# Rayhane-mamah/Tacotron-2

Hardware: NVIDIA H100
Metric: wavenet_train_audio_samples_per_sec (higher is better)
Workload: dtype bf16

## Files before the change

### tacotron-2_b200/csrc/t2_gemm.cu

```cuda
#include <stdlib.h>
#include <mutex>

#include "t2_gemm.cuh"
#include "t2_gemm.h"

namespace t2 {

static long long* g_timing_buffer = nullptr;
void set_timing_buffer(long long* p) { g_timing_buffer = p; }

typedef CUresult (*EncodeTiledFn)(CUtensorMap*, CUtensorMapDataType, cuuint32_t, void*, const cuuint64_t*,
                                  const cuuint64_t*, const cuuint32_t*, const cuuint32_t*,
                                  CUtensorMapInterleave, CUtensorMapSwizzle, CUtensorMapL2promotion,
                                  CUtensorMapFloatOOBfill);

static EncodeTiledFn get_encode_fn() {
  static EncodeTiledFn fn = nullptr;
  static std::once_flag once;
  std::call_once(once, [] {
    void* p = nullptr;
    cudaDriverEntryPointQueryResult q;
    if (cudaGetDriverEntryPoint("cuTensorMapEncodeTiled", &p, cudaEnableDefault, &q) == cudaSuccess &&
        q == cudaDriverEntryPointSuccess)
      fn = reinterpret_cast<EncodeTiledFn>(p);
// ... 110 lines not shown
    T2_REQUIRE(mc > 0, T2_ERR_UNSUPPORTED_SHAPE, "act_gemm: clusters of %d CTAs cannot be scheduled on this device", cs);
  }
  T2_CHECK_CUDA(cudaLaunchKernelEx(&cfg, act_gemm_kernel<EPI, BN>, g));
  t2_count_launch();
  return T2_OK;
}

int make_gemm_args(int epi, int BN, const ActGemmCall& c, GemmArgs& g, dim3& grid, int& cs) {
  T2_REQUIRE(c.na >= 1 && c.na <= 4 && c.nseg >= 1 && c.nseg <= kMaxSeg, T2_ERR_INVALID_ARG,
             "act_gemm: bad map/segment count (%d, %d)", c.na, c.nseg);
  T2_REQUIRE(c.cluster == 0 || c.cluster == 1 || c.cluster == 2 || c.cluster == 4 || c.cluster == 8, T2_ERR_INVALID_ARG,
             "act_gemm: cluster size must be 0 (default), 1, 2, 4 or 8 (got %d)", c.cluster);
  int ktot = 0;
  for (int s = 0; s < c.nseg; ++s) {
    T2_REQUIRE(c.seg[s].map >= 0 && c.seg[s].map < c.na && c.seg[s].nkb > 0 && c.seg[s].nlayers > 0,
               T2_ERR_INVALID_ARG, "act_gemm: bad segment %d", s);
    ktot += c.seg[s].nkb * c.seg[s].nlayers * kBK;
  }
  T2_REQUIRE(c.w_k0 + ktot <= ((c.wK + kBK - 1) / kBK) * kBK, T2_ERR_INVALID_ARG,
             "act_gemm: segments cover K=%d but packed weight has K=%d", ktot, c.wK);
  if (c.ksplit > 1) {
    T2_REQUIRE(epi == EPI_TOUT && c.ksplit * kBK <= ktot, T2_ERR_INVALID_ARG,
               "act_gemm: split-K needs an atomically accumulating epilogue and at least one k-block per slice");
    const bool use0 = c.epi.ptr[0] && c.epi.i[0] > 0, use1 = c.epi.ptr[1] && c.epi.i[3] > c.epi.i[0];
    T2_REQUIRE((!use0 || c.epi.i[2] == 2) && (!use1 || c.epi.i[5] == 2), T2_ERR_INVALID_ARG,
               "act_gemm: split-K needs atomic accumulation (mode 2) into every destination in use (modes %d, %d)", c.epi.i[2],
               c.epi.i[5]);
  }
  memset(&g, 0, sizeof(g));
  for (int i = 0; i < 4; ++i) {
    int rc = encode_act_map(&g.amap[i], c.a[i < c.na ? i : 0], kBM);
    if (rc) return rc;
  }
  grid = dim3((c.T + kBM - 1) / kBM * c.B, c.n_tiles, c.ksplit > 1 ? c.ksplit : 1);
  cs = pick_cluster(BN, grid, c.cluster);
  int rc = encode_wt_map(&g.bmap, c.w, c.wN, c.wK, c.wL, BN / cs);
  if (rc) return rc;
  for (int s = 0; s < c.nseg; ++s) g.seg[s] = c.seg[s];
  g.nseg = c.nseg;
  g.T = c.T;
  g.tiles_per_b = (c.T + kBM - 1) / kBM;
  g.b_layer = c.w_layer;
  g.b_k0 = c.w_k0;
  g.dbg = g_timing_buffer;
  g.epi = c.epi;
  if (!c.epi.i[11]) {
    const void* outs[3] = {nullptr, nullptr, nullptr};
    int ldo = 0;
    if (epi == EPI_GATE) { outs[0] = c.epi.ptr[0]; outs[1] = c.epi.ptr[1]; outs[2] = c.epi.ptr[2]; ldo = c.epi.i[0]; }
    else if (epi == EPI_RES) { outs[0] = c.epi.ptr[1]; outs[1] = c.epi.ptr[2]; ldo = BN; }
    else if (epi == EPI_GATE_BWD) { outs[0] = c.epi.ptr[2]; ldo = 2 * c.epi.i[0]; }
    else if (epi == EPI_DX) { outs[0] = c.epi.ptr[1]; ldo = BN; }
    for (int i = 0; i < 3; ++i)
      if (outs[i]) {
        rc = encode_out_map(&g.omap[i], outs[i], ldo, c.T, c.B);
        if (rc) return rc;
      }
  }
  return T2_OK;
}

long long* take_timing_slice(long long n_slots) {
  long long* p = g_timing_buffer;
  if (p) g_timing_buffer = p + n_slots;
  return p;
}

int launch_act_gemm(int epi, int BN, const ActGemmCall& c, cudaStream_t stream, int* cluster_used) {
  GemmArgs g;
  dim3 grid;
  int cs = 1;
  const int rc = make_gemm_args(epi, BN, c, g, grid, cs);
  if (rc) return rc;
  if (cluster_used) *cluster_used = cs;
#define T2_CASE(E, N) \
  if (epi == E && BN == N) return launch_one<E, N>(g, grid, cs, stream);
  T2_CASE(EPI_GATE, 256)
  T2_CASE(EPI_RES, 128)
  T2_CASE(EPI_RES, 256)
  T2_CASE(EPI_BIAS_ACT, 128)
  T2_CASE(EPI_BIAS_ACT, 256)
  T2_CASE(EPI_CE, 256)
  T2_CASE(EPI_SCALE_RELUMASK, 128)
  T2_CASE(EPI_SCALE_RELUMASK, 256)
  T2_CASE(EPI_GATE_BWD, 128)
  T2_CASE(EPI_GATE_BWD, 256)
  T2_CASE(EPI_DX, 128)
  T2_CASE(EPI_DX, 256)
  T2_CASE(EPI_MOL, 32)
  T2_CASE(EPI_LSTM, 32)
  T2_CASE(EPI_TOUT, 32)
#undef T2_CASE
  return t2_set_error(T2_ERR_UNSUPPORTED_SHAPE, "act_gemm: no kernel for epilogue %d with BN=%d", epi, BN);
}

int launch_wgrad(const ActT* maps, int nmaps, const WgradTile* tiles_dev, int ntiles, float* out, int T,
                 int B, cudaStream_t stream) {
  T2_REQUIRE(nmaps >= 1 && nmaps <= 6 && ntiles >= 1, T2_ERR_INVALID_ARG, "wgrad: bad map/tile count");
  WgradArgs g;
  memset(&g, 0, sizeof(g));
  for (int i = 0; i < 6; ++i) {
    int rc = encode_act_map(&g.map[i], maps[i < nmaps ? i : 0], kBK);
    if (rc) return rc;
  }
  g.tiles = tiles_dev;
  g.out = out;
  g.T = T;
  g.B = B;
  static bool configured = false;
  if (!configured) {
    T2_CHECK_CUDA(cudaFuncSetAttribute(wgrad_gemm_kernel, cudaFuncAttributeMaxDynamicSharedMemorySize, kWgSmemBytes));
    configured = true;
  }
  cudaLaunchConfig_t cfg;
  memset(&cfg, 0, sizeof(cfg));
  cfg.gridDim = dim3(ntiles); cfg.blockDim = dim3(kGemmThreads); cfg.dynamicSmemBytes = kWgSmemBytes; cfg.stream = stream;
  cudaLaunchAttribute attr[1];
  attr[0].id = cudaLaunchAttributeProgrammaticStreamSerialization;
  attr[0].val.programmaticStreamSerializationAllowed = 1;
  cfg.attrs = attr; cfg.numAttrs = pdl_enabled() ? 1 : 0;
  T2_CHECK_CUDA(cudaLaunchKernelEx(&cfg, wgrad_gemm_kernel, g));
  t2_count_launch();
  return T2_OK;
}

void append_wgrad_tiles(std::vector<WgradTile>& v, const WgradTile& proto, int a_ch0, int Ca, int b_ch0, int Cb, long long out_off,
                        int ldc) {
  for (int m0 = 0; m0 < Ca; m0 += kWgBM)
    for (int n0 = 0; n0 < Cb; n0 += kWgBN) {
      WgradTile t;
      memset(&t, 0, sizeof(t));
      t.a_map = proto.a_map; t.a_ch0 = a_ch0 + m0; t.a_shift = proto.a_shift; t.a_layer = proto.a_layer;
      t.b_map = proto.b_map; t.b_ch0 = b_ch0 + n0; t.b_shift = proto.b_shift; t.b_layer = proto.b_layer;
      t.out_off = out_off + (long long)m0 * ldc + n0; t.ldc = ldc;
      t.m_valid = Ca - m0 < kWgBM ? Ca - m0 : kWgBM;
      t.n_valid = Cb - n0 < kWgBN ? Cb - n0 : kWgBN;
      t.scale = proto.scale; t.accumulate = proto.accumulate; t.div = proto.div;
      v.push_back(t);
    }
}

constexpr long long kChainTimeoutNs = 1000000000LL;

__device__ __forceinline__ int ld_acquire_gpu(const int* p) {
  int v;
  asm volatile("ld.acquire.gpu.global.b32 %0, [%1];" : "=r"(v) : "l"(p) : "memory");
  return v;
}
__device__ __forceinline__ void red_release_gpu_add(int* p, int v) {
  asm volatile("red.release.gpu.global.add.s32 [%0], %1;" ::"l"(p), "r"(v) : "memory");
}
__device__ __forceinline__ void fence_proxy_async_global() { asm volatile("fence.proxy.async.global;" ::: "memory"); }

template <int BN>
__device__ __forceinline__ void chain_init_barriers(uint8_t* smem) {
  using Cfg = ActGemmCfg<BN>;
  uint64_t* full_bar = reinterpret_cast<uint64_t*>(smem + Cfg::kPipeBytes + Cfg::kEpiBytes);
  for (int i = 0; i < Cfg::kStages; ++i) {
    mbar_init(&full_bar[i], 1);
    mbar_init(&full_bar[Cfg::kStages + i], kActEpiWarps);
  }
  fence_barrier_init();
}
template <int BN>
__device__ __forceinline__ void chain_inval_barriers(uint8_t* smem) {
  using Cfg = ActGemmCfg<BN>;
  uint64_t* full_bar = reinterpret_cast<uint64_t*>(smem + Cfg::kPipeBytes + Cfg::kEpiBytes);
  for (int i = 0; i < 2 * Cfg::kStages; ++i)
    asm volatile("mbarrier.inval.shared::cta.b64 [%0];" ::"r"(smem_u32(&full_bar[i])) : "memory");
}

template <bool FWD, int BN0, int BN1>
__global__ void __launch_bounds__(kActGemmThreads, 1) wn_chain_kernel(const __grid_constant__ ChainArgs a) {
  constexpr int E0 = FWD ? EPI_GATE : EPI_GATE_BWD, E1 = FWD ? EPI_RES : EPI_DX;
  using C0 = ActGemmCfg<BN0>;
  using C1 = ActGemmCfg<BN1>;
  static_assert(C0::kPipeBytes == C1::kPipeBytes && C0::kEpiBytes == C1::kEpiBytes && C0::kSmemBytes == C1::kSmemBytes,
                "both GEMMs of a chain share one shared-memory plan");
  extern __shared__ uint8_t smem_raw[];
  uint8_t* smem = reinterpret_cast<uint8_t*>((reinterpret_cast<uintptr_t>(smem_raw) + 1023) & ~uintptr_t(1023));
  __shared__ EpiArgs s_epi;
  __shared__ int s_ticket;
  int* done = a.ctr + 16;
  int* stop = a.ctr + 1;
  int prev_kind = -1;
  for (;;) {
    if (threadIdx.x == 0) {
      int t = atomicAdd(a.ctr, 1);
      if (t < a.n_tix && *reinterpret_cast<volatile int*>(stop) == 0) {
        long long* dbg = a.dbg ? a.dbg + size_t(t) * kDbgSlots : nullptr;
        const long long t_start = globaltimer_ns();
        if (dbg) { dbg[0] = t_start; dbg[3] = smid(); }
        const ChainTicket k = a.tix[t];
        for (int i = k.dep_lo; i <= k.dep_hi && t < a.n_tix; ++i)
          while (ld_acquire_gpu(done + i) < k.dep_target) {
            if (globaltimer_ns() - t_start > kChainTimeoutNs) {
              if (atomicExch(stop, 1) == 0) atomicAdd(a.err, 1);
              t = a.n_tix;
              break;
            }
            __nanosleep(32);
          }
        fence_proxy_async_global();
        if (dbg) dbg[1] = globaltimer_ns();
        EpiArgs e = a.args[k.kind * a.L + k.layer].epi;
        if (FWD && k.kind == 0 && !a.save) { e.ptr[0] = nullptr; e.ptr[1] = nullptr; }
        if (FWD && k.kind == 1) e.ptr[3] = const_cast<float*>(a.params) + reinterpret_cast<uintptr_t>(e.ptr[3]);
        if (k.kind == 1) { e.seed = a.seed; e.ptr[7] = const_cast<unsigned long long*>(a.d_step); }
        s_epi = e;
        if (prev_kind == 0) chain_inval_barriers<BN0>(smem);
        else if (prev_kind == 1) chain_inval_barriers<BN1>(smem);
        if (k.kind == 0) chain_init_barriers<BN0>(smem);
        else chain_init_barriers<BN1>(smem);
        prev_kind = k.kind;
      } else {
        t = a.n_tix;
      }
      s_ticket = t;
    }
    __syncthreads();
    const int t = s_ticket;
    if (t >= a.n_tix) break;
    const ChainTicket k = a.tix[t];
    const GemmArgs& g = a.args[k.kind * a.L + k.layer];
    int all_kb = 0;
    for (int s = 0; s < g.nseg; ++s) all_kb += g.seg[s].nkb * g.seg[s].nlayers;
    if ((threadIdx.x >> 5) == kActEpiWarps) {
      fence_proxy_async_global();
      asm volatile("fence.proxy.async.shared::cta;" ::: "memory");
    }
    if (k.kind == 0) act_gemm_tile<E0, BN0, true>(g, s_epi, smem, k.m, k.n, 0, all_kb, 1, 0, 1, nullptr);
    else act_gemm_tile<E1, BN1, true>(g, s_epi, smem, k.m, k.n, 0, all_kb, 1, 0, 1, nullptr);
    fence_proxy_async_global();
    __syncthreads();
    if (threadIdx.x == 0) {
      red_release_gpu_add(done + k.done, 1);
      if (a.dbg) a.dbg[size_t(t) * kDbgSlots + 2] = globaltimer_ns();
    }
  }
}

template <bool FWD, int BN0, int BN1>
int launch_chain_kernel(const ChainArgs& a, int grid, cudaStream_t st) {
  static bool configured = false;
  if (!configured) {
    T2_CHECK_CUDA(cudaFuncSetAttribute(wn_chain_kernel<FWD, BN0, BN1>, cudaFuncAttributeMaxDynamicSharedMemorySize,
                                       ActGemmCfg<BN0>::kSmemBytes));
    configured = true;
  }
  wn_chain_kernel<FWD, BN0, BN1><<<grid, kActGemmThreads, ActGemmCfg<BN0>::kSmemBytes, st>>>(a);
  t2_count_launch();
  T2_CHECK_CUDA(cudaGetLastError());
  return T2_OK;
}


int launch_wn_chain(bool fwd, int bn0, int bn1, const ChainArgs& a, int grid, cudaStream_t st) {
  if (fwd && bn0 == 256) return bn1 == 256 ? launch_chain_kernel<true, 256, 256>(a, grid, st) : launch_chain_kernel<true, 256, 128>(a, grid, st);
  if (!fwd && bn0 == 256) return bn1 == 256 ? launch_chain_kernel<false, 256, 256>(a, grid, st) : launch_chain_kernel<false, 256, 128>(a, grid, st);
  if (!fwd && bn0 == 128) return bn1 == 256 ? launch_chain_kernel<false, 128, 256>(a, grid, st) : launch_chain_kernel<false, 128, 128>(a, grid, st);
  return t2_set_error(T2_ERR_UNSUPPORTED_SHAPE, "layer chain: no kernel for %s with BN %d / %d", fwd ? "forward" : "backward", bn0, bn1);
}

}
```

### tacotron-2_b200/csrc/t2_gemm.cuh

```cuda
#pragma once
#include "t2_common.cuh"
#include "t2_gemm_types.h"

namespace t2 {

__device__ __forceinline__ void store_bf16x32(__nv_bfloat16* dst, const float (&v)[32]) {
  uint4* d = reinterpret_cast<uint4*>(dst);
#pragma unroll
  for (int q = 0; q < 4; ++q) {
    uint4 u;
    u.x = pack_bf16x2(v[q * 8 + 0], v[q * 8 + 1]);
    u.y = pack_bf16x2(v[q * 8 + 2], v[q * 8 + 3]);
    u.z = pack_bf16x2(v[q * 8 + 4], v[q * 8 + 5]);
    u.w = pack_bf16x2(v[q * 8 + 6], v[q * 8 + 7]);
    d[q] = u;
  }
}
__device__ __forceinline__ void load_bf16x32(const __nv_bfloat16* src, float (&v)[32]) {
  const uint4* s = reinterpret_cast<const uint4*>(src);
#pragma unroll
  for (int q = 0; q < 4; ++q) {
    uint4 u = __ldg(s + q);
    v[q * 8 + 0] = bf16lo(u.x); v[q * 8 + 1] = bf16hi(u.x);
    v[q * 8 + 2] = bf16lo(u.y); v[q * 8 + 3] = bf16hi(u.y);
// ... 718 lines not shown
  static __device__ __forceinline__ void run(const EpiArgs& e, const EpiCtx& c) {
    const int R = BN;
    const __nv_bfloat16* dxo = static_cast<const __nv_bfloat16*>(e.ptr[0]);
    const float rs = e.f[0], p = e.f[1];
    const float keep_inv = 1.f / (1.f - p);
    const unsigned long long seed = e.seed + (e.ptr[7] ? *static_cast<const unsigned long long*>(e.ptr[7]) : 0ull);
    const uint32_t hs = hash_seed(seed, uint32_t(e.i[1]));
    const size_t row = (size_t(c.b) * c.T + c.t) * R;
    if (BN == 256 && dxo) tile_fill_sw<kCoherent>(c.tile(1), dxo + c.row0 * BN + 128, BN, c.nrows, c);
#pragma unroll 1
    for (int gq = 0; gq < BN / 128; ++gq) {
      uint8_t* tile = c.tile(gq == 0 ? 2 : 1);
      const int cq = c.cg;
      const int j0 = gq * 128 + cq * 32;
      float acc[32], g[32];
      acc_ld32f(c.trow + j0, acc);
      if (p > 0.f) {
        const uint32_t thr = uint32_t(p * 65536.f);
#pragma unroll
        for (int j = 0; j < 32; j += 2) {
          const uint32_t h = hash_bits32(hs, (row + j0 + j) >> 1);
          acc[j] = (h & 0xFFFFu) >= thr ? acc[j] * keep_inv : 0.f;
          acc[j + 1] = (h >> 16) >= thr ? acc[j + 1] * keep_inv : 0.f;
        }
      }
      if (dxo) {
        stage_get_sw(tile, c.lane, cq, g);
#pragma unroll
        for (int j = 0; j < 32; ++j) acc[j] += rs * g[j];
      }
      stage_put_sw(tile, c.lane, cq, acc);
      tile_store(tile, c.omap + 0, gq * 128, c);
      if (e.ptr[2]) {
        const float cs = warp_colsum32(acc, c.lane);
        fx_add(static_cast<long long*>(e.ptr[2]) + j0 + colsum32_col(c.lane), cs * e.f[2]);
      }
    }
  }
};

template <>
struct Epilogue<EPI_LSTM, 32> {
  static __device__ __forceinline__ void run(const EpiArgs& e, const EpiCtx& c) {
    const int H = e.i[0], nb = e.i[1];
    float* ex = reinterpret_cast<float*>(c.smem_all);
    const int q = c.qbar - 1;
    if (c.cg == 0) {
      float v[32];
      acc_ld32f(c.trow, v);
#pragma unroll
      for (int j = 0; j < 32; ++j) ex[(q * 32 + c.lane) * 33 + j] = v[j];
    }
    asm volatile("bar.sync 5, 512;\n" ::: "memory");
    const float* pre = static_cast<const float*>(e.ptr[0]);
    const float* bias = static_cast<const float*>(e.ptr[1]);
    const float* c_prev = static_cast<const float*>(e.ptr[2]);
    float* c_out = static_cast<float*>(e.ptr[3]);
    const __nv_bfloat16* h_prev = static_cast<const __nv_bfloat16*>(e.ptr[4]);
    __nv_bfloat16* h_state = static_cast<__nv_bfloat16*>(e.ptr[5]);
    __nv_bfloat16* h_out = static_cast<__nv_bfloat16*>(e.ptr[6]);
    __nv_bfloat16* gst = static_cast<__nv_bfloat16*>(e.ptr[7]);
    __nv_bfloat16* tst = static_cast<__nv_bfloat16*>(e.ptr[8]);
    const int* lens = static_cast<const int*>(e.ptr[9]);
    const unsigned long long seed = e.seed + (e.ptr[10] ? *static_cast<const unsigned long long*>(e.ptr[10]) : 0ull);
    const uint32_t hs_c = hash_seed(seed, uint32_t(e.i[8]) * 2u), hs_h = hash_seed(seed, uint32_t(e.i[8]) * 2u + 1u);
    const float z = e.f[0];
    const int t = e.i[7];
    const int etid = (c.cg * 4 + q) * 32 + c.lane;
    const int u0 = c.m_tile * 32, b0 = c.n_tile * 32;
#pragma unroll 1
    for (int p = etid; p < 1024; p += 512) {
      const int bl = p >> 5, ul = p & 31;
      const int b = b0 + bl, u = u0 + ul;
      if (b >= nb || u >= H) continue;
      float zi = ex[(0 * 32 + ul) * 33 + bl], zj = ex[(1 * 32 + ul) * 33 + bl];
      float zf = ex[(2 * 32 + ul) * 33 + bl], zo = ex[(3 * 32 + ul) * 33 + bl];
      if (pre) {
        const float* pr = pre + size_t(b) * e.i[3];
        zi += pr[u]; zj += pr[H + u]; zf += pr[2 * H + u]; zo += pr[3 * H + u];
      }
      if (bias) { zi += bias[u]; zj += bias[H + u]; zf += bias[2 * H + u]; zo += bias[3 * H + u]; }
      float gi = sigmoidf_(zi), gj = tanhf_(zj), gf = sigmoidf_(zf + 1.f), go = sigmoidf_(zo);
      const float cp = c_prev[size_t(b) * H + u];
      const float hp = __bfloat162float(h_prev[size_t(b) * e.i[4] + u]);
      const float cn = gf * cp + gi * gj;
      const float tc = tanhf_(cn);
      const float hn = go * tc;
      const bool live = lens ? (t < lens[b]) : true;
      float cs, hsv, ho = hn;
      if (e.i[9]) {
        const uint64_t idx = (uint64_t(t) * nb + b) * H + u;
        cs = (z <= 0.f || hash_uniform32(hs_c, idx) >= z) ? cn : cp;
        hsv = (z <= 0.f || hash_uniform32(hs_h, idx) >= z) ? hn : hp;
      } else {
        cs = (1.f - z) * cn + z * cp;
        hsv = (1.f - z) * hn + z * hp;
      }
      float tcs = tc;
      if (!live) { cs = cp; hsv = hp; ho = 0.f; gi = gj = gf = go = 0.f; tcs = 0.f; }
      c_out[size_t(b) * H + u] = cs;
      h_state[size_t(b) * e.i[5] + u] = __float2bfloat16(hsv);
      h_out[size_t(b) * e.i[6] + u] = __float2bfloat16(ho);
      if (gst) {
        __nv_bfloat16* g = gst + size_t(b) * 4 * H;
        g[u] = __float2bfloat16(gi); g[H + u] = __float2bfloat16(gj);
        g[2 * H + u] = __float2bfloat16(gf); g[3 * H + u] = __float2bfloat16(go);
      }
      if (tst) tst[size_t(b) * H + u] = __float2bfloat16(tcs);
    }
  }
};

template <>
struct Epilogue<EPI_TOUT, 32> {
  static __device__ __forceinline__ void run(const EpiArgs& e, const EpiCtx& c) {
    if (c.cg != 0) return;
    const int k = c.t, nb = e.i[6];
    float v[32];
    acc_ld32f(c.trow, v);
    float* dst; int ld, acc, kk;
    if (k < e.i[0]) { dst = static_cast<float*>(e.ptr[0]); ld = e.i[1]; acc = e.i[2]; kk = k; }
    else if (k < e.i[3]) { dst = static_cast<float*>(e.ptr[1]); ld = e.i[4]; acc = e.i[5]; kk = k - e.i[0]; }
    else return;
    if (!dst) return;
#pragma unroll
    for (int j = 0; j < 32; ++j) {
      const int b = c.n_tile * 32 + j;
      if (b < nb) {
        float* d = dst + size_t(b) * ld + kk;
        if (acc == 2) atomicAdd(d, v[j]);
        else *d = acc ? *d + v[j] : v[j];
      }
    }
  }
};

template <int BN>
struct ActGemmCfg {
  static constexpr int kABytes = kBM * kBK * 2;
  static constexpr int kBBytes = BN * kBK * 2;
  static constexpr int kStageBytes = kABytes + kBBytes;
  static constexpr int kAccBytes = kBM * BN * 4;
  static constexpr int kEpiBytes = 4 * kSTileBytes;
  static constexpr int kTailBytes = 8 * kSTileBytes;
  static constexpr int kPipeBudget = 232448 - kEpiBytes - 1024  - 256 ;
  static constexpr int kStages = kPipeBudget / kStageBytes > 6 ? 6 : kPipeBudget / kStageBytes;
  static constexpr int kPipeBytes =
      kStages * kStageBytes > kAccBytes + kTailBytes ? kStages * kStageBytes : kAccBytes + kTailBytes;
  static constexpr int kSmemBytes = kPipeBytes + kEpiBytes + 1024 + 256;
  static_assert(kStages >= 2 && kPipeBytes <= kPipeBudget && kSmemBytes <= 232448, "shared memory budget");
  static_assert(kPipeBytes % 1024 == 0, "staging tiles must be aligned to the 1024-byte swizzle atom");
};

template <int EPI, int BN, bool kChain = false>
__device__ __forceinline__ void act_gemm_tile(const GemmArgs& g, const EpiArgs& epi, uint8_t* smem, int m_tile, int n_tile,
                                              int kb_lo, int kb_hi, uint32_t cs, uint32_t crank, uint16_t cmask, long long* dbg) {
  using Cfg = ActGemmCfg<BN>;
  constexpr int WN = BN / 2;
  float* acc_s = reinterpret_cast<float*>(smem);
  uint8_t* staging = smem + Cfg::kPipeBytes - Cfg::kTailBytes;
  uint64_t* full_bar = reinterpret_cast<uint64_t*>(smem + Cfg::kPipeBytes + Cfg::kEpiBytes);
  uint64_t* empty_bar = full_bar + Cfg::kStages;
  const int warp = threadIdx.x >> 5;
  const int b = m_tile / g.tiles_per_b;
  const int t0 = (m_tile - b * g.tiles_per_b) * kBM;
  const int total_kb = kb_hi - kb_lo;

  if (warp == kActEpiWarps) {
    if (elect_one()) {
      int stage = 0;
      uint32_t phase = 0;
      int kb_global = 0;
      for (int s = 0; s < g.nseg; ++s) {
        const Seg sg = g.seg[s];
        for (int l = 0; l < sg.nlayers; ++l) {
          for (int kb = 0; kb < sg.nkb; ++kb, ++kb_global) {
            if (kb_global < kb_lo || kb_global >= kb_hi) continue;
            mbar_wait(&empty_bar[stage], phase ^ 1);
            mbar_expect_tx(&full_bar[stage], Cfg::kStageBytes);
            uint8_t* sa = smem + stage * Cfg::kStageBytes;
            uint8_t* sb = sa + Cfg::kABytes;
            tma_load_4d(sa, &g.amap[sg.map], &full_bar[stage], sg.k0 + kb * kBK, t0 + sg.shift, b, sg.layer0 + l);
            if (cs == 1) {
              tma_load_3d(sb, &g.bmap, &full_bar[stage], g.b_k0 + kb_global * kBK, n_tile * BN, g.b_layer);
            } else {
              const int rows = BN / int(cs);
              tma_load_3d_mc(sb + crank * rows * (kBK * 2), &g.bmap, &full_bar[stage], g.b_k0 + kb_global * kBK,
                             n_tile * BN + int(crank) * rows, g.b_layer, cmask);
            }
            if (++stage == Cfg::kStages) { stage = 0; phase ^= 1; }
          }
        }
      }
    }
  } else {
    const int q = warp & 3;
    const int lane = threadIdx.x & 31;
    EpiCtx c;
    c.lane = lane;
    c.cg = warp >> 2;
    c.qbar = 1 + q;
    c.b = b; c.T = g.T;
    const int tw = t0 + q * 32;
    c.t = tw + c.lane;
    c.valid = c.t < g.T;
    c.row0 = size_t(b) * g.T + tw;
    c.nrows = g.T - tw < 0 ? 0 : (g.T - tw > 32 ? 32 : g.T - tw);
    c.stg = staging + q * kSTileBytes;
    c.smem_all = smem + Cfg::kAccBytes;
    c.m_tile = m_tile;
    c.omap = g.omap; c.tq = tw; c.sk = 0;
    c.n_tile = n_tile;
    constexpr bool kCoh = EPI == EPI_RES || EPI == EPI_DX;
    if constexpr (kCoh) Epilogue<EPI, BN>::template prefetch<kChain>(epi, c);
    else if constexpr (EpiHasPrefetch<EPI>::value) Epilogue<EPI, BN>::prefetch(epi, c);

    const int wg = warp >> 2, mh = wg >> 1, nh = wg & 1;
    float d[WN / 2];
#pragma unroll
    for (int i = 0; i < WN / 2; ++i) d[i] = 0.f;
    int stage = 0, prev = 0;
    uint32_t phase = 0;
    for (int kb = 0; kb < total_kb; ++kb) {
      mbar_wait(&full_bar[stage], phase);
      __syncwarp();
      if (dbg && kb == 0 && threadIdx.x == 0) dbg[2] = clock64();
      const uint32_t sa = smem_u32(smem + stage * Cfg::kStageBytes) + uint32_t(mh * 64 * 128);
      const uint32_t sb = smem_u32(smem + stage * Cfg::kStageBytes + Cfg::kABytes) + uint32_t(nh * WN * 128);
      const uint64_t adesc = make_gdesc_sw128(sa, 16, 1024);
      const uint64_t bdesc = make_gdesc_sw128(sb, 16, 1024);
      wgmma_fence();
      wgmma_fence_regs(d);
#pragma unroll
      for (int k = 0; k < kBK / 16; ++k)
        Wgmma<WN, 0, 0>::mma(d, adesc + uint64_t(k * 2), bdesc + uint64_t(k * 2), (kb > 0 || k > 0) ? 1u : 0u);
      wgmma_commit();
      wgmma_fence_regs(d);
      wgmma_wait<1>();
      if (kb > 0 && lane == 0) {
        if (cs == 1) mbar_arrive(&empty_bar[prev]);
        else for (uint32_t r = 0; r < cs; ++r) mbar_arrive_cluster(&empty_bar[prev], r);
      }
      prev = stage;
      if (++stage == Cfg::kStages) { stage = 0; phase ^= 1; }
    }
    wgmma_wait<0>();
    wgmma_fence_regs(d);
    if (dbg && threadIdx.x == 0) dbg[3] = clock64();
    asm volatile("bar.sync 6, 512;\n" ::: "memory");
    {
      const int r0 = mh * 64 + (warp & 3) * 16 + (lane >> 2);
#pragma unroll
      for (int j = 0; j < WN / 8; ++j)
#pragma unroll
        for (int i = 0; i < 2; ++i) {
          const int r = r0 + 8 * i, col = nh * WN + 8 * j + 2 * (lane & 3);
          *reinterpret_cast<float2*>(acc_s + r * BN + ((((col >> 2) ^ (r & 7)) << 2) | (col & 3))) =
              make_float2(d[4 * j + 2 * i], d[4 * j + 2 * i + 1]);
        }
    }
    asm volatile("bar.sync 6, 512;\n" ::: "memory");
    const int row = q * 32 + lane;
    c.trow = AccRow{acc_s + row * BN, 0, row & 7};
    if (dbg && threadIdx.x == 0) dbg[4] = clock64();
    if constexpr (kCoh) Epilogue<EPI, BN>::template run<kChain>(epi, c);
    else Epilogue<EPI, BN>::run(epi, c);
    if (dbg && threadIdx.x == 0) dbg[5] = clock64();
    tile_store_drain(c);
  }
}

template <int EPI, int BN>
__global__ void __launch_bounds__(kActGemmThreads, 1) act_gemm_kernel(const __grid_constant__ GemmArgs g) {
  using Cfg = ActGemmCfg<BN>;
  constexpr int WN = BN / 2;
  extern __shared__ uint8_t smem_raw[];
  uint8_t* smem = reinterpret_cast<uint8_t*>((reinterpret_cast<uintptr_t>(smem_raw) + 1023) & ~uintptr_t(1023));
  float* acc_s = reinterpret_cast<float*>(smem);
  uint8_t* staging = smem + Cfg::kPipeBytes - Cfg::kTailBytes;
  uint64_t* full_bar = reinterpret_cast<uint64_t*>(smem + Cfg::kPipeBytes + Cfg::kEpiBytes);
  uint64_t* empty_bar = full_bar + Cfg::kStages;

  const int warp = threadIdx.x >> 5;
  const int m_tile = blockIdx.x;
  const uint32_t cs = cluster_nctarank(), crank = cluster_ctarank();
  const uint16_t cmask = uint16_t((1u << cs) - 1u);
  long long* dbg = g.dbg ? g.dbg + ((size_t(blockIdx.z) * gridDim.y + blockIdx.y) * gridDim.x + blockIdx.x) * kDbgSlots : nullptr;
  if (dbg && threadIdx.x == 0) { dbg[0] = clock64(); dbg[8] = globaltimer_ns(); dbg[11] = smid(); }
  const int b = m_tile / g.tiles_per_b;
  const int t0 = (m_tile - b * g.tiles_per_b) * kBM;

  int all_kb = 0;
  for (int s = 0; s < g.nseg; ++s) all_kb += g.seg[s].nkb * g.seg[s].nlayers;
  const int kb_lo = int((long long)all_kb * blockIdx.z / gridDim.z), kb_hi = int((long long)all_kb * (blockIdx.z + 1) / gridDim.z);
  const int total_kb = kb_hi - kb_lo;

  if (warp == kActEpiWarps && elect_one()) {
    for (int i = 0; i < 4; ++i) tma_prefetch_desc(&g.amap[i]);
    tma_prefetch_desc(&g.bmap);
    for (int i = 0; i < Cfg::kStages; ++i) {
      mbar_init(&full_bar[i], 1);
      mbar_init(&empty_bar[i], kActEpiWarps * cs);
    }
    fence_barrier_init();
  }
  __syncthreads();
  if (cs > 1) cluster_sync_all();
  pdl_wait();
  pdl_launch_dependents();
  if (dbg && threadIdx.x == 0) { dbg[1] = clock64(); dbg[9] = globaltimer_ns(); }

  if (warp == kActEpiWarps) {
    if (elect_one()) {
      const int n_tile = blockIdx.y;
      int stage = 0;
      uint32_t phase = 0;
      int kb_global = 0;
      for (int s = 0; s < g.nseg; ++s) {
        const Seg sg = g.seg[s];
        for (int l = 0; l < sg.nlayers; ++l) {
          for (int kb = 0; kb < sg.nkb; ++kb, ++kb_global) {
            if (kb_global < kb_lo || kb_global >= kb_hi) continue;
            mbar_wait(&empty_bar[stage], phase ^ 1);
            mbar_expect_tx(&full_bar[stage], Cfg::kStageBytes);
            uint8_t* sa = smem + stage * Cfg::kStageBytes;
            uint8_t* sb = sa + Cfg::kABytes;
            tma_load_4d(sa, &g.amap[sg.map], &full_bar[stage], sg.k0 + kb * kBK, t0 + sg.shift, b, sg.layer0 + l);
            if (cs == 1) {
              tma_load_3d(sb, &g.bmap, &full_bar[stage], g.b_k0 + kb_global * kBK, n_tile * BN, g.b_layer);
            } else {
              const int rows = BN / int(cs);
              tma_load_3d_mc(sb + crank * rows * (kBK * 2), &g.bmap, &full_bar[stage], g.b_k0 + kb_global * kBK,
                             n_tile * BN + int(crank) * rows, g.b_layer, cmask);
            }
            if (++stage == Cfg::kStages) { stage = 0; phase ^= 1; }
          }
        }
      }
    }
  } else {
    const int q = warp & 3;
    const int lane = threadIdx.x & 31;
    EpiCtx c;
    c.lane = lane;
    c.cg = warp >> 2;
    c.qbar = 1 + q;
    c.b = b; c.T = g.T;
    const int tw = t0 + q * 32;
    c.t = tw + c.lane;
    c.valid = c.t < g.T;
    c.row0 = size_t(b) * g.T + tw;
    c.nrows = g.T - tw < 0 ? 0 : (g.T - tw > 32 ? 32 : g.T - tw);
    c.stg = staging + q * kSTileBytes;
    c.smem_all = smem + Cfg::kAccBytes;
    c.m_tile = m_tile;
    c.omap = g.omap; c.tq = tw; c.sk = 0;
    c.n_tile = blockIdx.y;
    if constexpr (EpiHasPrefetch<EPI>::value) Epilogue<EPI, BN>::prefetch(g.epi, c);

    const int wg = warp >> 2, mh = wg >> 1, nh = wg & 1;
    float d[WN / 2];
#pragma unroll
    for (int i = 0; i < WN / 2; ++i) d[i] = 0.f;
    int stage = 0, prev = 0;
    uint32_t phase = 0;
    for (int kb = 0; kb < total_kb; ++kb) {
      mbar_wait(&full_bar[stage], phase);
      __syncwarp();
      if (dbg && kb == 0 && threadIdx.x == 0) dbg[2] = clock64();
      const uint32_t sa = smem_u32(smem + stage * Cfg::kStageBytes) + uint32_t(mh * 64 * 128);
      const uint32_t sb = smem_u32(smem + stage * Cfg::kStageBytes + Cfg::kABytes) + uint32_t(nh * WN * 128);
      const uint64_t adesc = make_gdesc_sw128(sa, 16, 1024);
      const uint64_t bdesc = make_gdesc_sw128(sb, 16, 1024);
      wgmma_fence();
      wgmma_fence_regs(d);
#pragma unroll
      for (int k = 0; k < kBK / 16; ++k)
        Wgmma<WN, 0, 0>::mma(d, adesc + uint64_t(k * 2), bdesc + uint64_t(k * 2), (kb > 0 || k > 0) ? 1u : 0u);
      wgmma_commit();
      wgmma_fence_regs(d);
      wgmma_wait<1>();
      if (kb > 0 && lane == 0) {
        if (cs == 1) mbar_arrive(&empty_bar[prev]);
        else for (uint32_t r = 0; r < cs; ++r) mbar_arrive_cluster(&empty_bar[prev], r);
      }
      prev = stage;
      if (++stage == Cfg::kStages) { stage = 0; phase ^= 1; }
    }
    wgmma_wait<0>();
    wgmma_fence_regs(d);
    if (dbg && threadIdx.x == 0) dbg[3] = clock64();
    asm volatile("bar.sync 6, 512;\n" ::: "memory");
    {
      const int r0 = mh * 64 + (warp & 3) * 16 + (lane >> 2);
#pragma unroll
      for (int j = 0; j < WN / 8; ++j)
#pragma unroll
        for (int i = 0; i < 2; ++i) {
          const int r = r0 + 8 * i, col = nh * WN + 8 * j + 2 * (lane & 3);
          *reinterpret_cast<float2*>(acc_s + r * BN + ((((col >> 2) ^ (r & 7)) << 2) | (col & 3))) =
              make_float2(d[4 * j + 2 * i], d[4 * j + 2 * i + 1]);
        }
    }
    asm volatile("bar.sync 6, 512;\n" ::: "memory");
    const int row = q * 32 + lane;
    c.trow = AccRow{acc_s + row * BN, 0, row & 7};
    if (dbg && threadIdx.x == 0) dbg[4] = clock64();
    Epilogue<EPI, BN>::run(g.epi, c);
    if (dbg && threadIdx.x == 0) dbg[5] = clock64();
    tile_store_drain(c);
  }
  __syncthreads();
  if (dbg && threadIdx.x == 0) { dbg[6] = clock64(); dbg[10] = globaltimer_ns(); }
  if (cs > 1) cluster_sync_all();
}

constexpr int kWgBM = 128;
constexpr int kWgBN = 256;
constexpr int kWgStages = 4;
constexpr int kWgStageBytes = 6 * (kBK * 128);
constexpr int kWgSmemBytes = kWgStages * kWgStageBytes + 1024 + 256;
static_assert(kWgSmemBytes <= 232448, "shared memory budget");
// ... 102 lines not shown
```

Measured before the change: 3.729 million.

## Overlap next chain ticket claim and TMA loads with current tile epilogue

Restructures the persistent WaveNet chain kernel so the producer warp claims the next ticket, waits on its dependencies and issues its TMA loads while the consumer warpgroups are still running the current tile's MMA and epilogue. Barriers are initialised once, with per-kind rings and a ring-free/ready handshake through double-buffered shared slots, replacing the per-ticket __syncthreads and barrier re-init. This is meant to hide the dependency spin and pipeline fill between tiles. It adds handshake complexity and a risk of ordering bugs, since the shared epilogue args are overwritten only after ring_free.

```diff
diff --git a/tacotron-2_b200/csrc/t2_gemm.cu b/tacotron-2_b200/csrc/t2_gemm.cu
--- a/tacotron-2_b200/csrc/t2_gemm.cu
+++ b/tacotron-2_b200/csrc/t2_gemm.cu
@@ -286,22 +286,41 @@
 }
 __device__ __forceinline__ void fence_proxy_async_global() { asm volatile("fence.proxy.async.global;" ::: "memory"); }
 
-template <int BN>
-__device__ __forceinline__ void chain_init_barriers(uint8_t* smem) {
-  using Cfg = ActGemmCfg<BN>;
-  uint64_t* full_bar = reinterpret_cast<uint64_t*>(smem + Cfg::kPipeBytes + Cfg::kEpiBytes);
-  for (int i = 0; i < Cfg::kStages; ++i) {
-    mbar_init(&full_bar[i], 1);
-    mbar_init(&full_bar[Cfg::kStages + i], kActEpiWarps);
-  }
-  fence_barrier_init();
-}
-template <int BN>
-__device__ __forceinline__ void chain_inval_barriers(uint8_t* smem) {
-  using Cfg = ActGemmCfg<BN>;
-  uint64_t* full_bar = reinterpret_cast<uint64_t*>(smem + Cfg::kPipeBytes + Cfg::kEpiBytes);
-  for (int i = 0; i < 2 * Cfg::kStages; ++i)
-    asm volatile("mbarrier.inval.shared::cta.b64 [%0];" ::"r"(smem_u32(&full_bar[i])) : "memory");
+struct ChainSlot {
+  ChainTicket k;
+  EpiArgs e;
+  int t;
+  RingPos pos;
+};
+
+template <bool FWD>
+__device__ __forceinline__ void chain_claim(const ChainArgs& a, ChainSlot& s) {
+  int* done = a.ctr + 16;
+  int* stop = a.ctr + 1;
+  int t = atomicAdd(a.ctr, 1);
+  if (t >= a.n_tix || *reinterpret_cast<volatile int*>(stop) != 0) { s.t = a.n_tix; return; }
+  long long* dbg = a.dbg ? a.dbg + size_t(t) * kDbgSlots : nullptr;
+  const long long t_start = globaltimer_ns();
+  if (dbg) { dbg[0] = t_start; dbg[3] = smid(); }
+  const ChainTicket k = a.tix[t];
+  for (int i = k.dep_lo; i <= k.dep_hi && t < a.n_tix; ++i)
+    while (ld_acquire_gpu(done + i) < k.dep_target) {
+      if (globaltimer_ns() - t_start > kChainTimeoutNs) {
+        if (atomicExch(stop, 1) == 0) atomicAdd(a.err, 1);
+        t = a.n_tix;
+        break;
+      }
+      __nanosleep(32);
+    }
+  fence_proxy_async_global();
+  if (dbg) dbg[1] = globaltimer_ns();
+  EpiArgs e = a.args[k.kind * a.L + k.layer].epi;
+  if (FWD && k.kind == 0 && !a.save) { e.ptr[0] = nullptr; e.ptr[1] = nullptr; }
+  if (FWD && k.kind == 1) e.ptr[3] = const_cast<float*>(a.params) + reinterpret_cast<uintptr_t>(e.ptr[3]);
+  if (k.kind == 1) { e.seed = a.seed; e.ptr[7] = const_cast<unsigned long long*>(a.d_step); }
+  s.k = k;
+  s.e = e;
+  s.t = t;
 }
 
 template <bool FWD, int BN0, int BN1>
@@ -311,65 +330,79 @@
   using C1 = ActGemmCfg<BN1>;
   static_assert(C0::kPipeBytes == C1::kPipeBytes && C0::kEpiBytes == C1::kEpiBytes && C0::kSmemBytes == C1::kSmemBytes,
                 "both GEMMs of a chain share one shared-memory plan");
+  constexpr bool kOneRing = BN0 == BN1;
+  constexpr int kBars = 2 * C0::kStages + (kOneRing ? 0 : 2 * C1::kStages) + 3;
+  static_assert(kBars * 8 <= 256, "stage, ring_free and slot barriers fit the barrier block");
   extern __shared__ uint8_t smem_raw[];
   uint8_t* smem = reinterpret_cast<uint8_t*>((reinterpret_cast<uintptr_t>(smem_raw) + 1023) & ~uintptr_t(1023));
+  __shared__ ChainSlot s_slot[2];
   __shared__ EpiArgs s_epi;
-  __shared__ int s_ticket;
-  int* done = a.ctr + 16;
-  int* stop = a.ctr + 1;
-  int prev_kind = -1;
-  for (;;) {
+  __shared__ int s_pub[2];
+  uint64_t* bar0 = reinterpret_cast<uint64_t*>(smem + C0::kPipeBytes + C0::kEpiBytes);
+  uint64_t* bar1 = kOneRing ? bar0 : bar0 + 2 * C0::kStages;
+  uint64_t* ring_free = bar1 + 2 * C1::kStages;
+  uint64_t* ready = ring_free + 1;
+  const int warp = threadIdx.x >> 5;
+  if (threadIdx.x == 0) {
+    for (int i = 0; i < C0::kStages; ++i) {
+      mbar_init(&bar0[i], 1);
+      mbar_init(&bar0[C0::kStages + i], kActEpiWarps);
+    }
+    if (!kOneRing)
+      for (int i = 0; i < C1::kStages; ++i) {
+        mbar_init(&bar1[i], 1);
+        mbar_init(&bar1[C1::kStages + i], kActEpiWarps);
+      }
+    mbar_init(ring_free, kActEpiWarps);
+    mbar_init(&ready[0], 1);
+    mbar_init(&ready[1], 1);
+    fence_barrier_init();
+  }
+  __syncthreads();
+
+  if (warp == kActEpiWarps) {
+    if (!elect_one()) return;
+    RingPos p0{0, 0}, p1{0, 0};
+    chain_claim<FWD>(a, s_slot[0]);
+    int i = 0;
+    for (; s_slot[i & 1].t < a.n_tix; ++i) {
+      ChainSlot& s = s_slot[i & 1];
+      const ChainTicket k = s.k;
+      const GemmArgs& g = a.args[k.kind * a.L + k.layer];
+      RingPos& p = (k.kind == 0 || kOneRing) ? p0 : p1;
+      s.pos = p;
+      if (i > 0) mbar_wait(ring_free, (i - 1) & 1);
+      s_epi = s.e;
+      mbar_arrive(&ready[i & 1]);
+      fence_proxy_async();
+      if (k.kind == 0) chain_tile_load<BN0>(g, smem, bar0, bar0 + C0::kStages, k.m, k.n, p);
+      else chain_tile_load<BN1>(g, smem, bar1, bar1 + C1::kStages, k.m, k.n, p);
+      chain_claim<FWD>(a, s_slot[(i + 1) & 1]);
+    }
+    mbar_arrive(&ready[i & 1]);
+    return;
+  }
+
+  for (int i = 0;; ++i) {
+    mbar_wait(&ready[i & 1], (i >> 1) & 1);
+    const ChainSlot& s = s_slot[i & 1];
+    const int t = s.t;
+    if (t >= a.n_tix) break;
+    const int kind = s.k.kind, m = s.k.m, n = s.k.n;
+    const RingPos pos = s.pos;
+    const GemmArgs& g = a.args[kind * a.L + s.k.layer];
+    if (threadIdx.x == 0) { s_pub[0] = t; s_pub[1] = s.k.done; }
+    long long* first_mma = a.dbg && threadIdx.x == 0 ? a.dbg + size_t(t) * kDbgSlots + 4 : nullptr;
+    if (kind == 0) chain_tile_mma<E0, BN0>(g, s_epi, smem, bar0, bar0 + C0::kStages, ring_free, m, n, pos, first_mma);
+    else chain_tile_mma<E1, BN1>(g, s_epi, smem, bar1, bar1 + C1::kStages, ring_free, m, n, pos, first_mma);
+    if ((warp >> 2) == 0 && (threadIdx.x & 31) == 0) {
+      bulk_wait_all();
+      fence_proxy_async_global();
+    }
+    asm volatile("bar.sync 7, 512;\n" ::: "memory");
     if (threadIdx.x == 0) {
-      int t = atomicAdd(a.ctr, 1);
-      if (t < a.n_tix && *reinterpret_cast<volatile int*>(stop) == 0) {
-        long long* dbg = a.dbg ? a.dbg + size_t(t) * kDbgSlots : nullptr;
-        const long long t_start = globaltimer_ns();
-        if (dbg) { dbg[0] = t_start; dbg[3] = smid(); }
-        const ChainTicket k = a.tix[t];
-        for (int i = k.dep_lo; i <= k.dep_hi && t < a.n_tix; ++i)
-          while (ld_acquire_gpu(done + i) < k.dep_target) {
-            if (globaltimer_ns() - t_start > kChainTimeoutNs) {
-              if (atomicExch(stop, 1) == 0) atomicAdd(a.err, 1);
-              t = a.n_tix;
-              break;
-            }
-            __nanosleep(32);
-          }
-        fence_proxy_async_global();
-        if (dbg) dbg[1] = globaltimer_ns();
-        EpiArgs e = a.args[k.kind * a.L + k.layer].epi;
-        if (FWD && k.kind == 0 && !a.save) { e.ptr[0] = nullptr; e.ptr[1] = nullptr; }
-        if (FWD && k.kind == 1) e.ptr[3] = const_cast<float*>(a.params) + reinterpret_cast<uintptr_t>(e.ptr[3]);
-        if (k.kind == 1) { e.seed = a.seed; e.ptr[7] = const_cast<unsigned long long*>(a.d_step); }
-        s_epi = e;
-        if (prev_kind == 0) chain_inval_barriers<BN0>(smem);
-        else if (prev_kind == 1) chain_inval_barriers<BN1>(smem);
-        if (k.kind == 0) chain_init_barriers<BN0>(smem);
-        else chain_init_barriers<BN1>(smem);
-        prev_kind = k.kind;
-      } else {
-        t = a.n_tix;
-      }
-      s_ticket = t;
-    }
-    __syncthreads();
-    const int t = s_ticket;
-    if (t >= a.n_tix) break;
-    const ChainTicket k = a.tix[t];
-    const GemmArgs& g = a.args[k.kind * a.L + k.layer];
-    int all_kb = 0;
-    for (int s = 0; s < g.nseg; ++s) all_kb += g.seg[s].nkb * g.seg[s].nlayers;
-    if ((threadIdx.x >> 5) == kActEpiWarps) {
-      fence_proxy_async_global();
-      asm volatile("fence.proxy.async.shared::cta;" ::: "memory");
-    }
-    if (k.kind == 0) act_gemm_tile<E0, BN0, true>(g, s_epi, smem, k.m, k.n, 0, all_kb, 1, 0, 1, nullptr);
-    else act_gemm_tile<E1, BN1, true>(g, s_epi, smem, k.m, k.n, 0, all_kb, 1, 0, 1, nullptr);
-    fence_proxy_async_global();
-    __syncthreads();
-    if (threadIdx.x == 0) {
-      red_release_gpu_add(done + k.done, 1);
-      if (a.dbg) a.dbg[size_t(t) * kDbgSlots + 2] = globaltimer_ns();
+      red_release_gpu_add(a.ctr + 16 + s_pub[1], 1);
+      if (a.dbg) a.dbg[size_t(s_pub[0]) * kDbgSlots + 2] = globaltimer_ns();
     }
   }
 }
diff --git a/tacotron-2_b200/csrc/t2_gemm.cuh b/tacotron-2_b200/csrc/t2_gemm.cuh
--- a/tacotron-2_b200/csrc/t2_gemm.cuh
+++ b/tacotron-2_b200/csrc/t2_gemm.cuh
@@ -894,122 +894,120 @@
   static_assert(kPipeBytes % 1024 == 0, "staging tiles must be aligned to the 1024-byte swizzle atom");
 };
 
-template <int EPI, int BN, bool kChain = false>
-__device__ __forceinline__ void act_gemm_tile(const GemmArgs& g, const EpiArgs& epi, uint8_t* smem, int m_tile, int n_tile,
-                                              int kb_lo, int kb_hi, uint32_t cs, uint32_t crank, uint16_t cmask, long long* dbg) {
+struct RingPos {
+  int stage;
+  uint32_t phase;
+};
+
+template <int BN>
+__device__ __forceinline__ void chain_tile_load(const GemmArgs& g, uint8_t* smem, uint64_t* full_bar, uint64_t* empty_bar,
+                                                int m_tile, int n_tile, RingPos& pos) {
+  using Cfg = ActGemmCfg<BN>;
+  const int b = m_tile / g.tiles_per_b;
+  const int t0 = (m_tile - b * g.tiles_per_b) * kBM;
+  int kb_global = 0;
+  for (int s = 0; s < g.nseg; ++s) {
+    const Seg sg = g.seg[s];
+    for (int l = 0; l < sg.nlayers; ++l) {
+      for (int kb = 0; kb < sg.nkb; ++kb, ++kb_global) {
+        mbar_wait(&empty_bar[pos.stage], pos.phase ^ 1);
+        mbar_expect_tx(&full_bar[pos.stage], Cfg::kStageBytes);
+        uint8_t* sa = smem + pos.stage * Cfg::kStageBytes;
+        uint8_t* sb = sa + Cfg::kABytes;
+        tma_load_4d(sa, &g.amap[sg.map], &full_bar[pos.stage], sg.k0 + kb * kBK, t0 + sg.shift, b, sg.layer0 + l);
+        tma_load_3d(sb, &g.bmap, &full_bar[pos.stage], g.b_k0 + kb_global * kBK, n_tile * BN, g.b_layer);
+        if (++pos.stage == Cfg::kStages) { pos.stage = 0; pos.phase ^= 1; }
+      }
+    }
+  }
+}
+
+template <int EPI, int BN>
+__device__ __forceinline__ void chain_tile_mma(const GemmArgs& g, const EpiArgs& epi, uint8_t* smem, uint64_t* full_bar,
+                                               uint64_t* empty_bar, uint64_t* ring_free, int m_tile, int n_tile, RingPos pos,
+                                               long long* first_mma) {
   using Cfg = ActGemmCfg<BN>;
   constexpr int WN = BN / 2;
   float* acc_s = reinterpret_cast<float*>(smem);
   uint8_t* staging = smem + Cfg::kPipeBytes - Cfg::kTailBytes;
-  uint64_t* full_bar = reinterpret_cast<uint64_t*>(smem + Cfg::kPipeBytes + Cfg::kEpiBytes);
-  uint64_t* empty_bar = full_bar + Cfg::kStages;
   const int warp = threadIdx.x >> 5;
   const int b = m_tile / g.tiles_per_b;
   const int t0 = (m_tile - b * g.tiles_per_b) * kBM;
-  const int total_kb = kb_hi - kb_lo;
-
-  if (warp == kActEpiWarps) {
-    if (elect_one()) {
-      int stage = 0;
-      uint32_t phase = 0;
-      int kb_global = 0;
-      for (int s = 0; s < g.nseg; ++s) {
-        const Seg sg = g.seg[s];
-        for (int l = 0; l < sg.nlayers; ++l) {
-          for (int kb = 0; kb < sg.nkb; ++kb, ++kb_global) {
-            if (kb_global < kb_lo || kb_global >= kb_hi) continue;
-            mbar_wait(&empty_bar[stage], phase ^ 1);
-            mbar_expect_tx(&full_bar[stage], Cfg::kStageBytes);
-            uint8_t* sa = smem + stage * Cfg::kStageBytes;
-            uint8_t* sb = sa + Cfg::kABytes;
-            tma_load_4d(sa, &g.amap[sg.map], &full_bar[stage], sg.k0 + kb * kBK, t0 + sg.shift, b, sg.layer0 + l);
-            if (cs == 1) {
-              tma_load_3d(sb, &g.bmap, &full_bar[stage], g.b_k0 + kb_global * kBK, n_tile * BN, g.b_layer);
-            } else {
-              const int rows = BN / int(cs);
-              tma_load_3d_mc(sb + crank * rows * (kBK * 2), &g.bmap, &full_bar[stage], g.b_k0 + kb_global * kBK,
-                             n_tile * BN + int(crank) * rows, g.b_layer, cmask);
-            }
-            if (++stage == Cfg::kStages) { stage = 0; phase ^= 1; }
-          }
-        }
-      }
-    }
-  } else {
-    const int q = warp & 3;
-    const int lane = threadIdx.x & 31;
-    EpiCtx c;
-    c.lane = lane;
-    c.cg = warp >> 2;
-    c.qbar = 1 + q;
-    c.b = b; c.T = g.T;
-    const int tw = t0 + q * 32;
-    c.t = tw + c.lane;
-    c.valid = c.t < g.T;
-    c.row0 = size_t(b) * g.T + tw;
-    c.nrows = g.T - tw < 0 ? 0 : (g.T - tw > 32 ? 32 : g.T - tw);
-    c.stg = staging + q * kSTileBytes;
-    c.smem_all = smem + Cfg::kAccBytes;
-    c.m_tile = m_tile;
-    c.omap = g.omap; c.tq = tw; c.sk = 0;
-    c.n_tile = n_tile;
-    constexpr bool kCoh = EPI == EPI_RES || EPI == EPI_DX;
-    if constexpr (kCoh) Epilogue<EPI, BN>::template prefetch<kChain>(epi, c);
-    else if constexpr (EpiHasPrefetch<EPI>::value) Epilogue<EPI, BN>::prefetch(epi, c);
-
-    const int wg = warp >> 2, mh = wg >> 1, nh = wg & 1;
-    float d[WN / 2];
-#pragma unroll
-    for (int i = 0; i < WN / 2; ++i) d[i] = 0.f;
-    int stage = 0, prev = 0;
-    uint32_t phase = 0;
-    for (int kb = 0; kb < total_kb; ++kb) {
-      mbar_wait(&full_bar[stage], phase);
-      __syncwarp();
-      if (dbg && kb == 0 && threadIdx.x == 0) dbg[2] = clock64();
-      const uint32_t sa = smem_u32(smem + stage * Cfg::kStageBytes) + uint32_t(mh * 64 * 128);
-      const uint32_t sb = smem_u32(smem + stage * Cfg::kStageBytes + Cfg::kABytes) + uint32_t(nh * WN * 128);
-      const uint64_t adesc = make_gdesc_sw128(sa, 16, 1024);
-      const uint64_t bdesc = make_gdesc_sw128(sb, 16, 1024);
-      wgmma_fence();
-      wgmma_fence_regs(d);
-#pragma unroll
-      for (int k = 0; k < kBK / 16; ++k)
-        Wgmma<WN, 0, 0>::mma(d, adesc + uint64_t(k * 2), bdesc + uint64_t(k * 2), (kb > 0 || k > 0) ? 1u : 0u);
-      wgmma_commit();
-      wgmma_fence_regs(d);
-      wgmma_wait<1>();
-      if (kb > 0 && lane == 0) {
-        if (cs == 1) mbar_arrive(&empty_bar[prev]);
-        else for (uint32_t r = 0; r < cs; ++r) mbar_arrive_cluster(&empty_bar[prev], r);
-      }
-      prev = stage;
-      if (++stage == Cfg::kStages) { stage = 0; phase ^= 1; }
-    }
-    wgmma_wait<0>();
+  int total_kb = 0;
+  for (int s = 0; s < g.nseg; ++s) total_kb += g.seg[s].nkb * g.seg[s].nlayers;
+
+  const int q = warp & 3;
+  const int lane = threadIdx.x & 31;
+  EpiCtx c;
+  c.lane = lane;
+  c.cg = warp >> 2;
+  c.qbar = 1 + q;
+  c.b = b; c.T = g.T;
+  const int tw = t0 + q * 32;
+  c.t = tw + c.lane;
+  c.valid = c.t < g.T;
+  c.row0 = size_t(b) * g.T + tw;
+  c.nrows = g.T - tw < 0 ? 0 : (g.T - tw > 32 ? 32 : g.T - tw);
+  c.stg = staging + q * kSTileBytes;
+  c.smem_all = smem + Cfg::kAccBytes;
+  c.m_tile = m_tile;
+  c.omap = g.omap; c.tq = tw; c.sk = 0;
+  c.n_tile = n_tile;
+  constexpr bool kCoh = EPI == EPI_RES || EPI == EPI_DX;
+  if constexpr (kCoh) Epilogue<EPI, BN>::template prefetch<true>(epi, c);
+  else if constexpr (EpiHasPrefetch<EPI>::value) Epilogue<EPI, BN>::prefetch(epi, c);
+
+  const int wg = warp >> 2, mh = wg >> 1, nh = wg & 1;
+  float d[WN / 2];
+#pragma unroll
+  for (int i = 0; i < WN / 2; ++i) d[i] = 0.f;
+  if (first_mma) {
+    mbar_wait(&full_bar[pos.stage], pos.phase);
+    *first_mma = globaltimer_ns();
+  }
+  int prev = 0;
+  for (int kb = 0; kb < total_kb; ++kb) {
+    mbar_wait(&full_bar[pos.stage], pos.phase);
+    __syncwarp();
+    const uint32_t sa = smem_u32(smem + pos.stage * Cfg::kStageBytes) + uint32_t(mh * 64 * 128);
+    const uint32_t sb = smem_u32(smem + pos.stage * Cfg::kStageBytes + Cfg::kABytes) + uint32_t(nh * WN * 128);
+    const uint64_t adesc = make_gdesc_sw128(sa, 16, 1024);
+    const uint64_t bdesc = make_gdesc_sw128(sb, 16, 1024);
+    wgmma_fence();
     wgmma_fence_regs(d);
-    if (dbg && threadIdx.x == 0) dbg[3] = clock64();
-    asm volatile("bar.sync 6, 512;\n" ::: "memory");
-    {
-      const int r0 = mh * 64 + (warp & 3) * 16 + (lane >> 2);
-#pragma unroll
-      for (int j = 0; j < WN / 8; ++j)
-#pragma unroll
-        for (int i = 0; i < 2; ++i) {
-          const int r = r0 + 8 * i, col = nh * WN + 8 * j + 2 * (lane & 3);
-          *reinterpret_cast<float2*>(acc_s + r * BN + ((((col >> 2) ^ (r & 7)) << 2) | (col & 3))) =
-              make_float2(d[4 * j + 2 * i], d[4 * j + 2 * i + 1]);
-        }
-    }
-    asm volatile("bar.sync 6, 512;\n" ::: "memory");
-    const int row = q * 32 + lane;
-    c.trow = AccRow{acc_s + row * BN, 0, row & 7};
-    if (dbg && threadIdx.x == 0) dbg[4] = clock64();
-    if constexpr (kCoh) Epilogue<EPI, BN>::template run<kChain>(epi, c);
-    else Epilogue<EPI, BN>::run(epi, c);
-    if (dbg && threadIdx.x == 0) dbg[5] = clock64();
-    tile_store_drain(c);
-  }
+#pragma unroll
+    for (int k = 0; k < kBK / 16; ++k)
+      Wgmma<WN, 0, 0>::mma(d, adesc + uint64_t(k * 2), bdesc + uint64_t(k * 2), (kb > 0 || k > 0) ? 1u : 0u);
+    wgmma_commit();
+    wgmma_fence_regs(d);
+    wgmma_wait<1>();
+    if (kb > 0 && lane == 0) mbar_arrive(&empty_bar[prev]);
+    prev = pos.stage;
+    if (++pos.stage == Cfg::kStages) { pos.stage = 0; pos.phase ^= 1; }
+  }
+  wgmma_wait<0>();
+  wgmma_fence_regs(d);
+  if (lane == 0) mbar_arrive(&empty_bar[prev]);
+  asm volatile("bar.sync 6, 512;\n" ::: "memory");
+  {
+    const int r0 = mh * 64 + (warp & 3) * 16 + (lane >> 2);
+#pragma unroll
+    for (int j = 0; j < WN / 8; ++j)
+#pragma unroll
+      for (int i = 0; i < 2; ++i) {
+        const int r = r0 + 8 * i, col = nh * WN + 8 * j + 2 * (lane & 3);
+        *reinterpret_cast<float2*>(acc_s + r * BN + ((((col >> 2) ^ (r & 7)) << 2) | (col & 3))) =
+            make_float2(d[4 * j + 2 * i], d[4 * j + 2 * i + 1]);
+      }
+  }
+  asm volatile("bar.sync 6, 512;\n" ::: "memory");
+  const int row = q * 32 + lane;
+  c.trow = AccRow{acc_s + row * BN, 0, row & 7};
+  if constexpr (kCoh) Epilogue<EPI, BN>::template run<true>(epi, c);
+  else Epilogue<EPI, BN>::run(epi, c);
+  if (c.cg == 0 && lane == 0) bulk_wait_read<0>();
+  __syncwarp();
+  if (lane == 0) mbar_arrive(ring_free);
 }
 
 template <int EPI, int BN>
```

Result: faster. 3.872 million, median of 6 (+3.8%).
